# BlueAnon/BD-BNN

Measured on AMD Instinct MI355X. Metric: train_images_per_sec, higher is better.
Workload: dtype bf16; 1 GPU; model=resnet18_bdbnn, global_batch=2048, image=3x224x224, kurtosis=True, parallelism=dp1

## Files before the change

### bdbnn_amd/csrc/api.h

```cpp
#pragma once
#include <hip/hip_runtime.h>
#include <cstdint>

constexpr int BDBNN_MAX_TENSORS = 64;

struct TensorListArg {
  const float* ptr[BDBNN_MAX_TENSORS];
  int64_t numel[BDBNN_MAX_TENSORS];
  int n;
};

struct PtrList { float* ptr[BDBNN_MAX_TENSORS]; };

constexpr int64_t BDBNN_CHUNK_ELEMS = 32 * 1024;

constexpr int bdbnn_bn_sum_rows(int act_kind) {
  return act_kind == 3 ? 4 : 3;
}

extern "C" {

void bdbnn_sign_pack(const void* x, uint32_t* out, int64_t pixels, int C,
                     int CW, bool bf16, hipStream_t stream);
void bdbnn_binsign_decode(const void* x, void* y, int64_t n, bool in_bf16,
// ... 91 lines not shown
                             int64_t n, int C, int act_kind, bool bf16,
                             hipStream_t stream);
void bdbnn_bn_fold_sums(const float* sums32, float* sums, int n,
                        hipStream_t stream);
void bdbnn_bn_act_bwd_apply(const void* dy, const void* z, const void* x,
                            const float* mean, const float* invstd,
                            const float* gamma, const float* a,
                            const float* sums, void* dx, void* dskip,
                            int64_t n, int C, int act_kind, float inv_n,
                            bool bf16, hipStream_t stream);
void bdbnn_bn_act_eval(const void* x, const void* skip, const float* rm,
                       const float* rv, const float* gamma,
                       const float* beta, const float* a, const float* b1,
                       const float* b2, void* out, int64_t n, int C,
                       int act_kind, float eps, bool bf16,
                       hipStream_t stream);
void bdbnn_bn_fold(const float* gamma, const float* beta, const float* rm,
                   const float* rv, const float* b1, float* sc, float* sh,
                   int C, float eps, hipStream_t stream);

void bdbnn_bn_relu_maxpool_fwd(
    const void* x, const float* mean, const float* invstd,
    const float* gamma, const float* beta, void* out, unsigned char* idx,
    uint32_t* xpk, uint32_t* mpk, int N, int C, int H, int W, int Ho, int Wo,
    int ks, int stride, int pad, bool bf16, hipStream_t stream);
void bdbnn_bn_relu_maxpool_bwd_reduce(
    const void* dy, const unsigned char* idx, const void* x,
    const float* mean, const float* invstd, const float* gamma,
    const float* beta, float* sums32, float* sums, int N, int C, int H,
    int W, int Ho, int Wo, int ks, int stride, int pad, bool bf16,
    hipStream_t stream);
void bdbnn_bn_relu_maxpool_bwd_apply(
    const void* dy, const unsigned char* idx, const void* x,
    const float* mean, const float* invstd, const float* gamma,
    const float* beta, const float* sums, void* dx, int N, int C, int H,
    int W, int Ho, int Wo, int ks, int stride, int pad, bool bf16,
    hipStream_t stream);

int bdbnn_dgrad2_supported(int H, int W, int C, int K);
int bdbnn_conv_dgrad2(const void* g, const void* wd, const uint32_t* mp,
                      const void* x, void* dx, const void* accp, int mode,
                      float t, float k, int N, int H, int W, int C, int K,
                      hipStream_t stream);
void bdbnn_dgrad_wdec(const uint32_t* wp, const float* alpha, void* wd,
                      int C, int K, int nt, hipStream_t stream);
int bdbnn_wgrad2_nslab(int N, int H, int W, int C, int K);
int bdbnn_conv_wgrad2(const void* g, const uint64_t* xcp, float* dwT, int N,
                      int H, int W, int C, int K, hipStream_t stream);
void bdbnn_repack_cplane(const uint32_t* xp, uint64_t* xcp, int NH, int W,
                         int C, int CW, bool parity, hipStream_t stream);
void bdbnn_wgrad_finish(const float* dwT, const float* w, float* dw, int C,
                        int K, int T, int nslab, hipStream_t stream);

int bdbnn_s2_kernels_can_run(int H, int W, int C, int K, int ks);
int bdbnn_dgrad2_s2_supported(int H, int W, int C, int K, int ks);
int bdbnn_conv_dgrad2_s2(const void* g, const void* wd, const uint32_t* mp,
                         const void* x, void* dx, const void* accp, int ks,
                         int mode, float t, float k, int N, int H, int W,
                         int C, int K, hipStream_t stream);
int bdbnn_wgrad2_s2_nslab(int N, int H, int W, int C, int K, int ks);
int bdbnn_conv_wgrad2_s2(const void* g, const uint64_t* planes, float* dwT,
                         int ks, int N, int H, int W, int C, int K,
                         hipStream_t stream);

void bdbnn_kurtosis_fwd(const TensorListArg* lists,
                        const int* block_tensor_dev,
                        const int64_t* block_off_dev, int n_blocks,
                        double* mom_dev, const float* targets, float* stats,
                        float* losses, float* kurts, hipStream_t stream);
void bdbnn_kurtosis_bwd(const TensorListArg* lists, const PtrList* gp,
                        const int* block_tensor_dev,
                        const int64_t* block_off_dev, int n_blocks,
                        const float* stats, const float* targets,
                        const float* gscale, hipStream_t stream);

void bdbnn_weight_kd_fwd(const TensorListArg* meta, const PtrList* ws,
                         const PtrList* wt, const int* bt, const int64_t* bo,
                         int n_blocks, double* out, hipStream_t stream);
void bdbnn_weight_kd_bwd(const TensorListArg* meta, const PtrList* wt,
                         const PtrList* grads, const int* bt,
                         const int64_t* bo, int n_blocks,
                         const float* gscale, hipStream_t stream);

void bdbnn_fused_sgd(const TensorListArg* meta, const PtrList* p,
                     const PtrList* g, const PtrList* buf, const int* bt,
                     const int64_t* bo, int n_blocks, float lr,
                     float momentum, float wd, hipStream_t stream);
void bdbnn_fused_adam(const TensorListArg* meta, const PtrList* p,
                      const PtrList* g, const PtrList* m1, const PtrList* m2,
                      const int* bt, const int64_t* bo, int n_blocks,
                      float lr, float beta1, float beta2, float eps,
                      float wd, float bc1, float bc2, hipStream_t stream);

}
```

### bdbnn_amd/csrc/bind.cpp

```cpp
#include <torch/extension.h>
#include <c10/hip/HIPStream.h>
#include <hip/hip_runtime.h>

#include <atomic>
#include <string>
#include <unordered_map>
#include <utility>
#include <vector>

#include "api.h"

namespace {

hipStream_t cur_stream() {
  return c10::hip::getCurrentHIPStream().stream();
}

bool is_bf16(const at::Tensor& t) { return t.scalar_type() == at::kBFloat16; }

void check_vec8(const at::Tensor& t, bool vec8_c, const char* name,
                const char* who) {
  TORCH_CHECK(t.is_cuda() && (t.scalar_type() == at::kBFloat16 ||
                              t.scalar_type() == at::kFloat),
              who, ": ", name, " must be a bf16 or fp32 CUDA tensor");
// ... 1138 lines not shown
                who, ": mask bitplane [...P...][C/32]");
  } else {
    check_act_bf16_cl(*x, N, C, H, W, who);
  }
  TORCH_CHECK(bdbnn_dgrad2_supported(H, W, (int)C, K) != 0, who,
              ": unsupported shape");
  at::Tensor ac = acc_as_bf16_cl(acc, N, C, H, W, who);
  auto dx = empty_dx(g, N, C, H, W);
  int rc = bdbnn_conv_dgrad2(
      g.data_ptr(), wd.data_ptr(),
      mp ? (const uint32_t*)mp->data_ptr<int>() : nullptr,
      x ? x->data_ptr() : nullptr, dx.data_ptr(),
      ac.defined() ? ac.data_ptr() : nullptr, (int)mode, (float)t, (float)k,
      N, H, W, (int)C, K, cur_stream());
  TORCH_CHECK(rc == 0, who, ": launch rejected the shape");
  return dx;
}

at::Tensor conv_dgrad2(const at::Tensor& g, const at::Tensor& wd,
                       const at::Tensor& mp, int64_t C,
                       const c10::optional<at::Tensor>& acc) {
  return conv_dgrad2_impl(g, wd, &mp, nullptr, C, 0, 0.0, 0.0, acc,
                          "conv_dgrad2");
}

at::Tensor conv_dgrad2_x(const at::Tensor& g, const at::Tensor& wd,
                         const at::Tensor& x, int64_t C, int64_t mode,
                         double t, double k,
                         const c10::optional<at::Tensor>& acc) {
  TORCH_CHECK(mode == 1 || mode == 2,
              "conv_dgrad2_x: mode must be 1 (approx) or 2 (EDE)");
  return conv_dgrad2_impl(g, wd, nullptr, &x, C, mode, t, k, acc,
                          "conv_dgrad2_x");
}

at::Tensor conv_wgrad2(const at::Tensor& g, const at::Tensor& xcp,
                       int64_t C) {
  check_grad_bf16_cl(g, "conv_wgrad2");
  int N = (int)g.size(0), K = (int)g.size(1);
  int H = (int)g.size(2), W = (int)g.size(3);
  TORCH_CHECK(xcp.dim() == 2 && xcp.size(0) == C &&
                  xcp.size(1) == (int64_t)N * H,
              "conv_wgrad2: c-plane bitplanes [C][N*H]");
  TORCH_CHECK(C % 64 == 0 && K % 64 == 0 && W <= 64,
              "conv_wgrad2: unsupported shape");
  int nslab = bdbnn_wgrad2_nslab(N, H, W, (int)C, K);
  TORCH_CHECK(nslab > 0, "conv_wgrad2: unsupported shape");
  auto dwT = at::empty({nslab, 9, C, K}, g.options().dtype(at::kFloat));
  int rc = bdbnn_conv_wgrad2(g.data_ptr(),
                             (const uint64_t*)xcp.data_ptr<int64_t>(),
                             dwT.data_ptr<float>(), N, H, W, (int)C, K,
                             cur_stream());
  TORCH_CHECK(rc == 0, "conv_wgrad2: launch rejected the shape");
  return dwT;
}


static bool s2_dims_sane(int64_t H, int64_t W, int64_t C, int64_t K) {
  return H >= 1 && W >= 1 && H <= (1 << 20) && C <= (1 << 20) &&
         K <= (1 << 20);
}
static bool dgrad2_s2_ok(int64_t H, int64_t W, int64_t C, int64_t K,
                         int64_t ks) {
  return s2_dims_sane(H, W, C, K) &&
         bdbnn_s2_kernels_can_run((int)H, (int)W, (int)C, (int)K,
                                  (int)ks) != 0;
}
static bool dgrad2_s2_routed(int64_t H, int64_t W, int64_t C, int64_t K,
                             int64_t ks) {
  return s2_dims_sane(H, W, C, K) &&
         bdbnn_dgrad2_s2_supported((int)H, (int)W, (int)C, (int)K,
                                   (int)ks) != 0;
}

at::Tensor conv_dgrad2_s2(const at::Tensor& g, const at::Tensor& wd,
                          int64_t H, int64_t W, int64_t C, int64_t mode,
                          const c10::optional<at::Tensor>& mp,
                          const c10::optional<at::Tensor>& x, double t,
                          double k, const c10::optional<at::Tensor>& acc) {
  const char* who = "conv_dgrad2_s2";
  check_grad_bf16_cl(g, who);
  int N = (int)g.size(0), K = (int)g.size(1);
  TORCH_CHECK(wd.is_cuda() && wd.dim() == 3 &&
                  wd.scalar_type() == at::kBFloat16 && wd.is_contiguous(),
              "conv_dgrad2_s2: wd must be contiguous bf16 [ks*ks][C][K]");
  TORCH_CHECK(wd.size(0) == 9 || wd.size(0) == 1,
              "conv_dgrad2_s2: wd.size(0) must be 9 (3x3) or 1 (1x1)");
  int ks = wd.size(0) == 9 ? 3 : 1;
  TORCH_CHECK(wd.size(1) == C && wd.size(2) == K,
              "conv_dgrad2_s2: wd must be [ks*ks][C][K] for this g and C");
  TORCH_CHECK(dgrad2_s2_ok(H, W, C, K, ks),
              "conv_dgrad2_s2: unsupported shape (H, W, C, K, ks)");
  int64_t Ho = (H + 1) / 2, Wo = (W + 1) / 2;
  TORCH_CHECK(g.size(2) == Ho && g.size(3) == Wo,
              "conv_dgrad2_s2: g spatial size must be the (Ho, Wo) implied "
              "by (H, W, ks)");
  TORCH_CHECK(mode >= 0 && mode <= 2,
              "conv_dgrad2_s2: mode must be 0 (clip-STE), 1 (approx) or 2 "
              "(EDE)");
  const uint32_t* mp_ptr = nullptr;
  const void* x_ptr = nullptr;
  if (mode == 0) {
    TORCH_CHECK(mp.has_value() && !x.has_value(),
                "conv_dgrad2_s2: mode 0 needs mp and x=None");
    TORCH_CHECK(mp->is_cuda() && mp->scalar_type() == at::kInt &&
                    mp->is_contiguous() && mp->size(-1) == C / 32 &&
// ... 198 lines not shown
  m.def("maxpool_bwd", &maxpool_bwd, "gather-based NHWC maxpool bwd");
  m.def("prelu_fwd", &prelu_fwd, "fused NHWC per-channel PReLU fwd");
  m.def("prelu_bwd", &prelu_bwd, "fused NHWC per-channel PReLU bwd");
  m.def("bn_act_fwd_train", &bn_act_fwd_train,
        "fused BN(+add)(+act) training forward -> [out, z, mean, invstd(, "
        "xpk, mpk)]; act_kind 3 (RPReLU) takes b1, b2 and stores u = z + b1 "
        "as z",
        py::arg("x"), py::arg("skip"), py::arg("gamma"), py::arg("beta"),
        py::arg("a"), py::arg("running_mean"), py::arg("running_var"),
        py::arg("momentum"), py::arg("eps"), py::arg("act_kind"),
        py::arg("pre_s1"), py::arg("pre_s2"), py::arg("want_pack"),
        py::arg("b1") = py::none(), py::arg("b2") = py::none());
  m.def("bn_act_bwd", &bn_act_bwd,
        "fused BN(+add)(+act) backward -> [dx, dskip, dgamma, dbeta, da]; "
        "act_kind 3 appends db1, db2");
  m.def("bn_act_eval", &bn_act_eval, "fused BN(+add)(+act) eval forward",
        py::arg("x"), py::arg("skip"), py::arg("gamma"), py::arg("beta"),
        py::arg("a"), py::arg("rm"), py::arg("rv"), py::arg("eps"),
        py::arg("act_kind"), py::arg("b1") = py::none(),
        py::arg("b2") = py::none());
  m.def("bn_relu_maxpool_fwd_train", &bn_relu_maxpool_fwd_train,
        "fused BN + ReLU + maxpool training forward -> [out, idx, mean, "
        "invstd(, xpk, mpk)]",
        py::arg("x"), py::arg("gamma"), py::arg("beta"),
        py::arg("running_mean"), py::arg("running_var"),
        py::arg("momentum"), py::arg("eps"), py::arg("ks"),
        py::arg("stride"), py::arg("pad"), py::arg("pre_s1") = py::none(),
        py::arg("pre_s2") = py::none(), py::arg("want_pack") = false);
  m.def("bn_relu_maxpool_bwd", &bn_relu_maxpool_bwd,
        "fused BN + ReLU + maxpool backward -> [dx, dgamma, dbeta]");
  m.def("conv_dgrad2", &conv_dgrad2,
        "MFMA bf16 dgrad v2: halo-staged 9-tap implicit GEMM with fused "
        "clip-STE mask (3x3/s1/p1); optional acc adds a same-shape "
        "skip-gradient tensor in the epilogue",
        py::arg("g"), py::arg("wd"), py::arg("mp"), py::arg("C"),
        py::arg("acc") = py::none());
  m.def("conv_dgrad2_x", &conv_dgrad2_x,
        "conv_dgrad2 with a value mask of the saved bf16 activation x in "
        "the epilogue: mode 1 = ReAct polynomial, 2 = EDE(t, k)",
        py::arg("g"), py::arg("wd"), py::arg("x"), py::arg("C"),
        py::arg("mode"), py::arg("t"), py::arg("k"),
        py::arg("acc") = py::none());
  m.def("dgrad_weight_decode", &dgrad_weight_decode,
        "packed bits -> mirrored transposed +-alpha bf16 [9][C][K]");
  m.def("dgrad2_supported",
        [](int64_t H, int64_t W, int64_t C, int64_t K) {
          return bdbnn_dgrad2_supported((int)H, (int)W, (int)C, (int)K) !=
                 0;
        },
        "shape support predicate for conv_dgrad2");
  m.def("conv_wgrad2", &conv_wgrad2,
        "MFMA bf16 wgrad v2: all-9-tap block GEMM from sign BITS "
        "(3x3/s1/p1) -> fp32 [9][C][K]");
  m.def("repack_cplane", &repack_cplane,
        "activation sign bits -> padded per-channel u64 row planes");
  m.def("wgrad_finish", &wgrad_finish,
        "dwT transpose to [K][C][3][3] + |w|<=1 STE mask, one pass");
  m.def("dgrad2_s2_supported",
        [](int64_t H, int64_t W, int64_t C, int64_t K, int64_t ks) {
          return dgrad2_s2_routed(H, W, C, K, ks);
        },
        "routing predicate of the stride-2 MFMA backward; H, W are the "
        "input (dx) size, ks in {3 (pad 1), 1 (pad 0)}; false also for "
        "the shapes the kernels run but lose on (3x3 with C >= 128 and "
        "K >= 256)",
        py::arg("H"), py::arg("W"), py::arg("C"), py::arg("K"),
        py::arg("ks"));
  m.def("conv_dgrad2_s2", &conv_dgrad2_s2,
        "MFMA bf16 dgrad of a 3x3/s2/p1 (wd [9][C][K]) or 1x1/s2/p0 (wd "
        "[1][C][K]) binary conv by pixel parity; mode 0 masks with the "
        "bitplane mp, modes 1/2 with the value mask of x; optional acc "
        "adds a same-shape skip-gradient tensor in the epilogue",
        py::arg("g"), py::arg("wd"), py::arg("H"), py::arg("W"),
        py::arg("C"), py::arg("mode"), py::arg("mp"), py::arg("x"),
        py::arg("t"), py::arg("k"), py::arg("acc") = py::none());
  m.def("dgrad_weight_decode_1x1", &dgrad_weight_decode_1x1,
        "packed 1x1 bits -> transposed +-alpha bf16 [1][C][K]");
  m.def("repack_cplane_s2", &repack_cplane_s2,
        "activation sign bits -> per-channel u64 row planes split by "
        "column parity (even columns low word, odd columns high word)",
        py::arg("xp"), py::arg("C"), py::arg("H"), py::arg("W"));
  m.def("conv_wgrad2_s2", &conv_wgrad2_s2,
        "MFMA bf16 wgrad of a 3x3/s2/p1 or 1x1/s2/p0 binary conv from the "
        "parity planes -> fp32 [nslab][ks*ks][C][K]",
        py::arg("g"), py::arg("planes"), py::arg("C"), py::arg("H"),
        py::arg("W"), py::arg("ks"));
  m.def("wgrad_finish_s2", &wgrad_finish_s2,
        "dwT slab sum + transpose to [K][C][ks][ks] + |w|<=1 STE mask");
  m.def("kurtosis_fwd", &kurtosis_fwd, "fused multi-tensor kurtosis fwd");
  m.def("kurtosis_bwd", &kurtosis_bwd, "fused multi-tensor kurtosis bwd");
  m.def("weight_kd_fwd", &weight_kd_fwd, "fused weight-space KD fwd");
  m.def("weight_kd_bwd", &weight_kd_bwd, "fused weight-space KD bwd");
  m.def("fused_sgd", &fused_sgd, "fused multi-tensor SGD-momentum step");
  m.def("fused_adam", &fused_adam, "fused multi-tensor Adam step");
}
```

### bdbnn_amd/csrc/conv_bwd.hip

```cpp
#include "conv_bwd_common.h"

#define DG2_BM 256
#define DG2_BN 64
#define DG2_BK 64

struct Dgrad2Params {
  int N, H, W, C, K;
  int bands_per_image;
  int total_slots;
  int CW;
};

template <int WP, int RB, int GB, bool ACC, int MODE>
__global__ __launch_bounds__(512, 2) void conv_dgrad2_kernel(
    const __bf16* __restrict__ g, const __bf16* __restrict__ wd,
    const uint32_t* __restrict__ mp, __bf16* __restrict__ dx,
    const __bf16* __restrict__ accp, const __bf16* __restrict__ xin,
    float et, float ek,
    Dgrad2Params p, int grid_m, int nb_m, int tiles_per_block) {
  constexpr int WH = WP + 2;
  constexpr int NHE = GB * (RB + 2) * WH;
  constexpr int PIECES = NHE * 8;
  constexpr int PPT = (PIECES + 511) / 512;

// ... 284 lines not shown
                                 float t, float k, int N, int H, int W,
                                 int C, int K, hipStream_t stream) {
  if (mode == 0)
    return dgrad2_launch<0>(g, wd, mp, dx, accp, nullptr, 0.f, 0.f, N, H, W,
                            C, K, stream);
  if (mode == 1)
    return dgrad2_launch<1>(g, wd, nullptr, dx, accp, x, 0.f, 0.f, N, H, W,
                            C, K, stream);
  if (mode == 2)
    return dgrad2_launch<2>(g, wd, nullptr, dx, accp, x, t, k, N, H, W, C,
                            K, stream);
  return -2;
}

template <int NT>
__global__ void dgrad_wdec_kernel(const uint32_t* __restrict__ wp,
                                  const float* __restrict__ alpha,
                                  __bf16* __restrict__ wd, int C, int K,
                                  int CW) {
  int64_t total = (int64_t)NT * C * (K / 8);
  GRID_STRIDE(i, total) {
    int k8 = int(i % (K / 8));
    int64_t rem = i / (K / 8);
    int c = NT == 1 ? int(rem) : int(rem % C);
    int t = NT == 1 ? 0 : int(rem / C);
    int tm = NT - 1 - t;
    int cw = c >> 5, cb = c & 31;
    __bf16 v[8];
#pragma unroll
    for (int j = 0; j < 8; ++j) {
      int k = k8 * 8 + j;
      uint32_t bits = wp[((int64_t)k * NT + tm) * CW + cw];
      float al = alpha[k];
      v[j] = (__bf16)((bits >> cb) & 1 ? -al : al);
    }
    *(uint4*)&wd[((int64_t)t * C + c) * K + k8 * 8] = *(uint4*)v;
  }
}

extern "C" void bdbnn_dgrad_wdec(const uint32_t* wp, const float* alpha,
                                 void* wd, int C, int K, int nt,
                                 hipStream_t stream) {
  int64_t total = (int64_t)nt * C * (K / 8);
  int blocks = (int)bd_min<int64_t>((total + 255) / 256, 4096);
  if (nt == 9)
    dgrad_wdec_kernel<9><<<blocks, 256, 0, stream>>>(wp, alpha, (__bf16*)wd,
                                                     C, K, C / 32);
  else
    dgrad_wdec_kernel<1><<<blocks, 256, 0, stream>>>(wp, alpha, (__bf16*)wd,
                                                     C, K, C / 32);
}


#define WG2_CHUNK 128
#define WG2_BC 64
#define WG2_BK 64

struct Wgrad2Params {
  int N, H, W, C, K;
  int bands_per_image;
  int total_slots;
  int total_chunks;
  int split;
  int nh_rows;
};

template <int WP, int RB, int GB>
__global__ __launch_bounds__(512, 2) void conv_wgrad2_kernel(
    const __bf16* __restrict__ g, const uint64_t* __restrict__ xcp,
    float* __restrict__ dwT, Wgrad2Params p, int grid_ck) {
  constexpr int XROWS = RB + 2;
  constexpr int XSTRIDE = GB * XROWS * WP + 8;
  constexpr int GSTRIDE = WG2_CHUNK + 8;
  constexpr int LGWP = WP == 8 ? 3 : WP == 16 ? 4 : WP == 32 ? 5 : 6;
  constexpr bool RING = (GB == 1);

  const int tid = threadIdx.x;
  int wg = blockIdx.x;
  const int ck = wg % grid_ck;
  const int split_id = wg / grid_ck;
  const int c_blk = ck % (p.C / WG2_BC);
  const int k_blk = ck / (p.C / WG2_BC);
  const int c0 = c_blk * WG2_BC, k0 = k_blk * WG2_BK;

  __shared__ __align__(16) __bf16 X[3 * WG2_BC * XSTRIDE];
  __shared__ __align__(16) __bf16 gT[2][WG2_BK * GSTRIDE];
  __shared__ __align__(16) __bf16 lut[256][8];
  __shared__ float red[4][32][32];
  constexpr int NBITS = WG2_BC * GB * XROWS;
  __shared__ uint64_t xbits[NBITS];
  __shared__ unsigned char xvalid[NBITS];

  wgrad2_fill_sign_lut(lut, tid);

  const int wid = tid >> 6, lane = tid & 63;
  const int qc = (wid >> 1) & 1, qk = wid & 1, ms_grp = wid >> 2;
  const int lrow = lane & 31, lhalf = lane >> 5;

  f32x16 acc[9];
#pragma unroll
  for (int t = 0; t < 9; ++t)
#pragma unroll
    for (int i = 0; i < 16; ++i) acc[t][i] = 0.f;

  const int cpb = (p.total_chunks + p.split - 1) / p.split;
  const int ch_lo = split_id * cpb;
  const int ch_hi = bd_min(ch_lo + cpb, p.total_chunks);
  const int n_chunks = ch_hi - ch_lo;
  int ch = ch_lo;

  const int sg_m = tid >> 2;
  const int sg_k16 = (tid & 3) * 16;
  uint4 greg[2];

#define G_LOAD(chunk)                                                     \
  {                                                                       \
    int band = sg_m / (RB * WP);                                          \
    int rem = sg_m - band * (RB * WP);                                    \
// ... 142 lines not shown
    const int y0m = RING ? u_pb[0] : 0;
    __syncthreads();
    if (cont) X_DECODE(ch, 2, RB)
    else X_DECODE(ch, 0, XROWS)
    if (more) {
      CHUNK_INFO(ch + 1);
      if (cont_n) BITS_LOAD(ch + 1, 2, RB)
      else BITS_LOAD(ch + 1, 0, XROWS)
      G_LOAD(ch + 1);
    }
    __syncthreads();

#pragma unroll
    for (int msl = 0; msl < 4; ++msl) {
      const int m16 = ms_grp * 64 + msl * 16;
      bf16x8 bfrag =
          *(const bf16x8*)&gT[gb][b_k * GSTRIDE + m16 + lhalf * 8];
      const int mstart = m16 + lhalf * 8;
      const int rl = mstart >> LGWP;
      const int band = rl / RB, rloc = rl - band * RB;
      const int xs = mstart & (WP - 1);
      int pl[3];
#pragma unroll
      for (int dy = 0; dy < 3; ++dy) {
        int v = RING ? y0m + rloc + dy : rloc + dy;
        if (RING && v >= XROWS) v -= XROWS;
        if (RING && v >= XROWS) v -= XROWS;
        pl[dy] = band * XROWS + v;
      }
#pragma unroll
      for (int t = 0; t < 9; ++t) {
        const int dy = t / 3, dxs = t - dy * 3;
        bf16x8 afrag = *(const bf16x8*)&X[(dxs * WG2_BC + a_c) * XSTRIDE +
                                          pl[dy] * WP + xs];
        acc[t] =
            __builtin_amdgcn_mfma_f32_32x32x16_bf16(afrag, bfrag, acc[t],
                                                    0, 0, 0);
      }
    }
    __syncthreads();
    if (more) {
      if (cont_n) BITS_WRITE(ch + 1, 2, RB)
      else BITS_WRITE(ch + 1, 0, XROWS)
      G_WRITE(gb ^ 1);
    }
    gb ^= 1;
    ++ch;
  }

  wgrad2_combine_store<9>(acc, red, dwT + (int64_t)split_id * 9 * p.C * p.K,
                          p.C, p.K, c0, k0, wid, lane);
}

template <class F>
static int wgrad2_class(int H, int W, F f) {
  if (W <= 8 && H <= 8) return f(BwdClass<8, 8, 2>{});
  if (W <= 16) return f(BwdClass<16, 8, 1>{});
  if (W <= 32) return f(BwdClass<32, 4, 1>{});
  return f(BwdClass<64, 2, 1>{});
}

static bool wgrad2_shape_ok(int W, int C, int K) {
  return !(C % 64 || K % 64 || W > 64);
}

template <class G>
static Wgrad2Params wgrad2_params(G, int N, int H, int W, int C, int K) {
  Wgrad2Params p;
  p.N = N; p.H = H; p.W = W; p.C = C; p.K = K;
  p.nh_rows = N * H;
  p.bands_per_image = (H + G::RB - 1) / G::RB;
  p.total_slots = N * p.bands_per_image;
  p.total_chunks = (p.total_slots + G::GB - 1) / G::GB;
  int grid_ck = (C / WG2_BC) * (K / WG2_BK);
  p.split = bd_min((256 + grid_ck - 1) / grid_ck, p.total_chunks);
  return p;
}

extern "C" int bdbnn_wgrad2_nslab(int N, int H, int W, int C, int K) {
  if (!wgrad2_shape_ok(W, C, K)) return -1;
  return wgrad2_class(H, W, [&](auto cls) {
    return wgrad2_params(cls, N, H, W, C, K).split;
  });
}

extern "C" int bdbnn_conv_wgrad2(const void* g, const uint64_t* xcp,
                                 float* dwT, int N, int H, int W, int C,
                                 int K, hipStream_t stream) {
  if (!wgrad2_shape_ok(W, C, K)) return -1;
  return wgrad2_class(H, W, [&](auto cls) {
    using G = decltype(cls);
    Wgrad2Params p = wgrad2_params(cls, N, H, W, C, K);
    int grid_ck = (C / WG2_BC) * (K / WG2_BK);
    dim3 grid(grid_ck * p.split);
    conv_wgrad2_kernel<G::WP, G::RB, G::GB><<<grid, 512, 0, stream>>>(
        (const __bf16*)g, xcp, dwT, p, grid_ck);
    return 0;
  });
}

template <bool PARITY>
__global__ void repack_cplane_kernel(const uint32_t* __restrict__ xp,
                                     uint64_t* __restrict__ xcp, int NH,
                                     int W, int C, int CW) {
  GRID_STRIDE(i, (int64_t)NH * CW) {
    int cw = int(i % CW);
    int64_t row = i / CW;
    const uint32_t* src = xp + (row * W) * CW + cw;
    uint64_t acc[32];
#pragma unroll
    for (int c = 0; c < 32; ++c) acc[c] = 0;
    for (int x = 0; x < W; ++x) {
      uint32_t word = src[(int64_t)x * CW];
      int pos = PARITY ? (x >> 1) + ((x & 1) << 5) : x;
#pragma unroll
      for (int c = 0; c < 32; ++c)
        acc[c] |= (uint64_t)((word >> c) & 1) << pos;
    }
#pragma unroll
    for (int c = 0; c < 32; ++c) {
      int cc = cw * 32 + c;
      if (cc < C) xcp[(int64_t)cc * NH + row] = acc[c];
    }
  }
}

extern "C" void bdbnn_repack_cplane(const uint32_t* xp, uint64_t* xcp,
                                    int NH, int W, int C, int CW,
                                    bool parity, hipStream_t stream) {
  int64_t total = (int64_t)NH * CW;
  int blocks = (int)bd_min<int64_t>((total + 255) / 256, 8192);
// ... 40 lines not shown
```

### bdbnn_amd/csrc/conv_bwd_common.h

```cpp
#pragma once
#include "common.h"
#include "act_masks.h"

typedef __attribute__((ext_vector_type(8))) __bf16 bf16x8;
typedef __attribute__((ext_vector_type(16))) float f32x16;

template <int WPV, int RBV, int GBV>
struct BwdClass {
  static constexpr int WP = WPV, RB = RBV, GB = GBV;
};

__device__ __forceinline__ int mfma32_cd_row(int reg, int half) {
  return (reg & 3) + 8 * (reg >> 2) + 4 * half;
}

__device__ __forceinline__ void wgrad2_fill_sign_lut(__bf16 (*lut)[8],
                                                     int tid) {
  for (int b = tid; b < 256; b += 512) {
#pragma unroll
    for (int j = 0; j < 8; ++j)
      lut[b][j] = (__bf16)(((b >> j) & 1) ? 1.f : -1.f);
  }
}

template <int NT>
__device__ __forceinline__ void wgrad2_combine_store(
    const f32x16 (&acc)[NT], float (*red)[32][32], float* __restrict__ slab,
    int C, int K, int c0, int k0, int wid, int lane) {
  const int quad = wid & 3, ms_grp = wid >> 2;
  const int qc = (wid >> 1) & 1, qk = wid & 1;
  const int lrow = lane & 31, lhalf = lane >> 5;
#pragma unroll
  for (int t = 0; t < NT; ++t) {
    __syncthreads();
    if (ms_grp == 1) {
#pragma unroll
      for (int reg = 0; reg < 16; ++reg)
        red[quad][mfma32_cd_row(reg, lhalf)][lrow] = acc[t][reg];
    }
    __syncthreads();
    if (ms_grp == 0) {
#pragma unroll
      for (int reg = 0; reg < 16; ++reg) {
        int row = mfma32_cd_row(reg, lhalf);
        float v = acc[t][reg] + red[quad][row][lrow];
        slab[((int64_t)t * C + c0 + qc * 32 + row) * K + k0 + qk * 32 +
             lrow] = v;
      }
    }
  }
}

template <int MODE>
__device__ __forceinline__ float dgrad2_value_mask(float x, float et,
                                                   float ekt) {
  static_assert(MODE == 1 || MODE == 2, "value mask: mode 1 or 2");
  if constexpr (MODE == 1) {
    return react_poly_mask(x);
  }
  float e = __expf(-2.f * fabsf(et * x));
  float d = 1.f + e;
  return ekt * __fdividef(4.f * e, d * d);
}
```

### bdbnn_amd/ops/binary_conv.py

```python

import os

import torch
import torch.nn as nn
import torch.nn.functional as F

from .binarize import binsign, weight_scale
from .. import _C

_CONV_STATS = os.environ.get("BDBNN_CONV_STATS", "0") == "1"
_MFMA_BWD = os.environ.get("BDBNN_MFMA_BWD", "1") != "0"
_MFMA_BWD_S2 = os.environ.get("BDBNN_MFMA_BWD_S2", "1") != "0"


def _act_grad_mask(x: torch.Tensor, mode: str, t, k) -> torch.Tensor:
    if t is not None and k is not None:
        th = torch.tanh(float(t) * x)
        return float(k) * float(t) * (1.0 - th * th)
    if mode == "approx":
        neg = (x >= -1) & (x < 0)
        pos = (x >= 0) & (x < 1)
        g = torch.zeros_like(x)
        g = torch.where(neg, 2.0 + 2.0 * x, g)
        g = torch.where(pos, 2.0 - 2.0 * x, g)
        return g
    return (x.abs() <= 1).to(x.dtype)


def _owned_route(nat, *, g_dtype, x_dtype, stride, padding, ks, H_in, W_in,
                 H_out, W_out, C, K, mask_mode, valmask):
    if not _MFMA_BWD or (valmask and mask_mode == 0):
        return None
    if g_dtype != torch.bfloat16 or x_dtype != torch.bfloat16:
        return None
    if (ks, stride, padding) == (3, 1, 1):
        return "s1" if nat.dgrad2_supported(H_out, W_out, C, K) else None
    if _MFMA_BWD_S2 and stride == 2 and (ks, padding) in ((3, 1), (1, 0)):
        return "s2" if nat.dgrad2_s2_supported(H_in, W_in, C, K, ks) else None
    return None


def _owned_backward(nat, route, g, w, xp, wp, alpha, C, mode, mp, x, t, k,
                    acc):
    s2 = route == "s2"
    H, W, ks = xp.shape[1], xp.shape[2], w.shape[2]
    wd = (nat.dgrad_weight_decode_1x1 if ks == 1
          else nat.dgrad_weight_decode)(wp, alpha, C)
    if s2:
        dx = nat.conv_dgrad2_s2(g, wd, H, W, C, mode, mp, x, t, k, acc)
        planes = nat.repack_cplane_s2(xp, C, H, W)
        dwT = nat.conv_wgrad2_s2(g, planes, C, H, W, ks)
        dw = nat.wgrad_finish_s2(dwT, w.float())
    else:
        dx = (nat.conv_dgrad2(g, wd, mp, C, acc) if mode == 0
              else nat.conv_dgrad2_x(g, wd, x, C, mode, t, k, acc))
        planes = nat.repack_cplane(xp, C, W)
        dwT = nat.conv_wgrad2(g, planes, C)
        dw = nat.wgrad_finish(dwT, w.float())
    return dx, dw


def _conv_backward(g, xb, wb, stride, padding):
    return torch.ops.aten.convolution_backward(
        g, xb, wb, None, [stride, stride], [padding, padding], [1, 1], False,
        [0, 0], 1, [True, True, False])[:2]


def _packed_fallback(nat, g, w, xp, mp, wp, alpha, C, x_dtype, stride,
                     padding):
    bf16 = g.dtype == torch.bfloat16
    xb = nat.decode_packed(xp, C, bf16)
    wb = nat.weight_decode(wp, alpha, C, bf16)
    dxb, dwb = _conv_backward(g, xb, wb, stride, padding)
    dx = nat.mask_mul_packed(dxb, mp, C, x_dtype == torch.bfloat16)
    return dx, nat.ste_mask_mul(dwb, w, 0, 0.0, 0.0)


def _value_fallback(g, x, w, stride, padding, act_mode, t, k):
    if not x.is_cuda:
        dxb, dwb = _conv_backward(g, binsign(x), weight_scale(w) * binsign(w),
                                  stride, padding)
        return (dxb * _act_grad_mask(x, act_mode, t, k),
                dwb * (w.abs() <= 1).to(w.dtype))
    nat = _C.native_required()
    xb = nat.binsign_decode(x, 1 if g.dtype == torch.bfloat16 else 0)
    wb = (weight_scale(w) * binsign(w)).to(g.dtype)
    dxb, dwb = _conv_backward(g, xb, wb, stride, padding)
    if t is not None and k is not None:
        mode_id, t, k = 2, float(t), float(k)
    else:
        mode_id, t, k = {"ste": 0, "approx": 1}[act_mode], 0.0, 0.0
    return (nat.ste_mask_mul(dxb, x, mode_id, t, k),
            nat.ste_mask_mul(dwb, w, 0, 0.0, 0.0))


class BinaryConvFunction(torch.autograd.Function):

    @staticmethod
    def forward(ctx, x, w, stride, padding, act_mode, t, k,
                want_stats=False, xp_pre=None, mp_pre=None, skip_cell=None):
        ctx.stride = stride
        ctx.padding = padding
        ctx.act_mode = act_mode
        ctx.t = t
        ctx.k = k
        ctx.packed = False
        ctx.valmask = False
        ctx.skip_cell = skip_cell
        if x.is_cuda:
            nat = _C.native_required()
# ... 154 lines not shown
```

### setup.py

```python

import os

from setuptools import setup

os.environ.setdefault("PYTORCH_ROCM_ARCH", "gfx950")

from torch.utils.cpp_extension import BuildExtension, CUDAExtension

ROOT = os.path.dirname(os.path.abspath(__file__))
CSRC = os.path.join(ROOT, "bdbnn_amd", "csrc")

sources = [os.path.join(CSRC, f) for f in (
    "bind.cpp",
    "pack.hip",
    "prelu.hip",
    "bn_act.hip",
    "bn_pool.hip",
    "pool.hip",
    "loss.hip",
    "conv_bwd.hip",
    "conv_bwd_s2.hip",
    "stem_conv.hip",
    "xnor_conv.hip",
    "xnor_conv_mfma.hip",
    "kurtosis.hip",
    "kd.hip",
    "optim.hip",
)]

setup(
    name="bdbnn_amd_native",
    ext_modules=[
        CUDAExtension(
            name="bdbnn_amd._native",
            sources=sources,
            extra_compile_args={
                "cxx": ["-O3", "-std=c++17"],
                "nvcc": ["-O3", "-std=c++17"],
            },
        )
    ],
    cmdclass={"build_ext": BuildExtension.with_options(no_python_abi_suffix=False)},
)
```

Before: 27670 images/s.

## Add pipelined wgrad v3 kernel reading NHWC sign plane with transposed LDS reads

Adds a new MFMA weight-gradient kernel for 3x3 stride-1 binary convs. It reads the packed NHWC sign bits directly, which removes the separate repack_cplane pass. It double-buffers the gradient tiles and the activation ring so global loads overlap MFMA work, and it uses ds_read_tr16 transposed LDS reads with a swizzled layout. Shared wgrad2 helpers move to the common header, and the new route is on by default for all supported widths. The cost is more LDS and register pressure in a new, untested kernel.

```diff
diff --git a/bdbnn_amd/csrc/api.h b/bdbnn_amd/csrc/api.h
--- a/bdbnn_amd/csrc/api.h
+++ b/bdbnn_amd/csrc/api.h
@@ -167,6 +167,11 @@
 void bdbnn_wgrad_finish(const float* dwT, const float* w, float* dw, int C,
                         int K, int T, int nslab, hipStream_t stream);
 
+int bdbnn_wgrad3_supported(int H, int W, int C, int K);
+int bdbnn_wgrad3_nslab(int N, int H, int W, int C, int K);
+int bdbnn_conv_wgrad3(const void* g, const uint32_t* xp, float* dwT, int N,
+                      int H, int W, int C, int K, hipStream_t stream);
+
 int bdbnn_s2_kernels_can_run(int H, int W, int C, int K, int ks);
 int bdbnn_dgrad2_s2_supported(int H, int W, int C, int K, int ks);
 int bdbnn_conv_dgrad2_s2(const void* g, const void* wd, const uint32_t* mp,
diff --git a/bdbnn_amd/csrc/bind.cpp b/bdbnn_amd/csrc/bind.cpp
--- a/bdbnn_amd/csrc/bind.cpp
+++ b/bdbnn_amd/csrc/bind.cpp
@@ -1214,6 +1214,29 @@
                              dwT.data_ptr<float>(), N, H, W, (int)C, K,
                              cur_stream());
   TORCH_CHECK(rc == 0, "conv_wgrad2: launch rejected the shape");
+  return dwT;
+}
+
+at::Tensor conv_wgrad3(const at::Tensor& g, const at::Tensor& xp,
+                       int64_t C) {
+  check_grad_bf16_cl(g, "conv_wgrad3");
+  int N = (int)g.size(0), K = (int)g.size(1);
+  int H = (int)g.size(2), W = (int)g.size(3);
+  TORCH_CHECK(C >= 64 && C % 64 == 0 && K % 64 == 0 && W <= 64,
+              "conv_wgrad3: unsupported shape");
+  TORCH_CHECK(xp.is_cuda() && xp.dim() == 4 &&
+                  xp.scalar_type() == at::kInt && xp.is_contiguous() &&
+                  xp.size(0) == N && xp.size(1) == H && xp.size(2) == W &&
+                  xp.size(3) == C / 32,
+              "conv_wgrad3: xp must be contiguous int32 [N][H][W][C/32]");
+  int nslab = bdbnn_wgrad3_nslab(N, H, W, (int)C, K);
+  TORCH_CHECK(nslab > 0, "conv_wgrad3: unsupported shape");
+  auto dwT = at::empty({nslab, 9, C, K}, g.options().dtype(at::kFloat));
+  int rc = bdbnn_conv_wgrad3(g.data_ptr(),
+                             (const uint32_t*)xp.data_ptr<int>(),
+                             dwT.data_ptr<float>(), N, H, W, (int)C, K,
+                             cur_stream());
+  TORCH_CHECK(rc == 0, "conv_wgrad3: launch rejected the shape");
   return dwT;
 }
 
@@ -1518,6 +1541,16 @@
   m.def("conv_wgrad2", &conv_wgrad2,
         "MFMA bf16 wgrad v2: all-9-tap block GEMM from sign BITS "
         "(3x3/s1/p1) -> fp32 [9][C][K]");
+  m.def("conv_wgrad3", &conv_wgrad3,
+        "MFMA bf16 wgrad v3: pipelined all-9-tap block GEMM from the NHWC "
+        "sign plane, transposed LDS reads (3x3/s1/p1) -> fp32 "
+        "[nslab][9][C][K]");
+  m.def("wgrad3_supported",
+        [](int64_t H, int64_t W, int64_t C, int64_t K) {
+          return bdbnn_wgrad3_supported((int)H, (int)W, (int)C, (int)K) !=
+                 0;
+        },
+        "shape predicate of the conv_wgrad3 route");
   m.def("repack_cplane", &repack_cplane,
         "activation sign bits -> padded per-channel u64 row planes");
   m.def("wgrad_finish", &wgrad_finish,
diff --git a/bdbnn_amd/csrc/conv_bwd.hip b/bdbnn_amd/csrc/conv_bwd.hip
--- a/bdbnn_amd/csrc/conv_bwd.hip
+++ b/bdbnn_amd/csrc/conv_bwd.hip
@@ -360,18 +360,6 @@
 }
 
 
-#define WG2_CHUNK 128
-#define WG2_BC 64
-#define WG2_BK 64
-
-struct Wgrad2Params {
-  int N, H, W, C, K;
-  int bands_per_image;
-  int total_slots;
-  int total_chunks;
-  int split;
-  int nh_rows;
-};
 
 template <int WP, int RB, int GB>
 __global__ __launch_bounds__(512, 2) void conv_wgrad2_kernel(
@@ -620,31 +608,6 @@
                           p.C, p.K, c0, k0, wid, lane);
 }
 
-template <class F>
-static int wgrad2_class(int H, int W, F f) {
-  if (W <= 8 && H <= 8) return f(BwdClass<8, 8, 2>{});
-  if (W <= 16) return f(BwdClass<16, 8, 1>{});
-  if (W <= 32) return f(BwdClass<32, 4, 1>{});
-  return f(BwdClass<64, 2, 1>{});
-}
-
-static bool wgrad2_shape_ok(int W, int C, int K) {
-  return !(C % 64 || K % 64 || W > 64);
-}
-
-template <class G>
-static Wgrad2Params wgrad2_params(G, int N, int H, int W, int C, int K) {
-  Wgrad2Params p;
-  p.N = N; p.H = H; p.W = W; p.C = C; p.K = K;
-  p.nh_rows = N * H;
-  p.bands_per_image = (H + G::RB - 1) / G::RB;
-  p.total_slots = N * p.bands_per_image;
-  p.total_chunks = (p.total_slots + G::GB - 1) / G::GB;
-  int grid_ck = (C / WG2_BC) * (K / WG2_BK);
-  p.split = bd_min((256 + grid_ck - 1) / grid_ck, p.total_chunks);
-  return p;
-}
-
 extern "C" int bdbnn_wgrad2_nslab(int N, int H, int W, int C, int K) {
   if (!wgrad2_shape_ok(W, C, K)) return -1;
   return wgrad2_class(H, W, [&](auto cls) {
diff --git a/bdbnn_amd/csrc/conv_bwd_common.h b/bdbnn_amd/csrc/conv_bwd_common.h
--- a/bdbnn_amd/csrc/conv_bwd_common.h
+++ b/bdbnn_amd/csrc/conv_bwd_common.h
@@ -51,6 +51,44 @@
   }
 }
 
+#define WG2_CHUNK 128
+#define WG2_BC 64
+#define WG2_BK 64
+
+struct Wgrad2Params {
+  int N, H, W, C, K;
+  int bands_per_image;
+  int total_slots;
+  int total_chunks;
+  int split;
+  int nh_rows;
+};
+
+template <class F>
+static int wgrad2_class(int H, int W, F f) {
+  if (W <= 8 && H <= 8) return f(BwdClass<8, 8, 2>{});
+  if (W <= 16) return f(BwdClass<16, 8, 1>{});
+  if (W <= 32) return f(BwdClass<32, 4, 1>{});
+  return f(BwdClass<64, 2, 1>{});
+}
+
+static inline bool wgrad2_shape_ok(int W, int C, int K) {
+  return !(C % 64 || K % 64 || W > 64);
+}
+
+template <class G>
+static Wgrad2Params wgrad2_params(G, int N, int H, int W, int C, int K) {
+  Wgrad2Params p;
+  p.N = N; p.H = H; p.W = W; p.C = C; p.K = K;
+  p.nh_rows = N * H;
+  p.bands_per_image = (H + G::RB - 1) / G::RB;
+  p.total_slots = N * p.bands_per_image;
+  p.total_chunks = (p.total_slots + G::GB - 1) / G::GB;
+  int grid_ck = (C / WG2_BC) * (K / WG2_BK);
+  p.split = bd_min((256 + grid_ck - 1) / grid_ck, p.total_chunks);
+  return p;
+}
+
 template <int MODE>
 __device__ __forceinline__ float dgrad2_value_mask(float x, float et,
                                                    float ekt) {
diff --git a/bdbnn_amd/csrc/conv_wgrad3.hip b/bdbnn_amd/csrc/conv_wgrad3.hip
--- /dev/null
+++ b/bdbnn_amd/csrc/conv_wgrad3.hip
@@ -0,0 +1,263 @@
+#include "conv_bwd_common.h"
+
+typedef __attribute__((ext_vector_type(4))) short wg3_s16x4;
+typedef __attribute__((ext_vector_type(8))) short wg3_s16x8;
+
+__device__ __forceinline__ int wg3_off(int pix, int cb) {
+  return pix * 128 + (cb ^ ((pix & 2) << 5));
+}
+
+__device__ __forceinline__ wg3_s16x4 wg3_tr_read(const char* base, int off) {
+  return __builtin_amdgcn_ds_read_tr16_b64_v4i16(
+      (__attribute__((address_space(3))) wg3_s16x4*)(base + off));
+}
+
+__device__ __forceinline__ bf16x8 wg3_frag(wg3_s16x4 lo, wg3_s16x4 hi) {
+  wg3_s16x8 v = __builtin_shufflevector(lo, hi, 0, 1, 2, 3, 4, 5, 6, 7);
+  return __builtin_bit_cast(bf16x8, v);
+}
+
+template <int WP, int RB, int GB>
+__device__ __forceinline__ void wg3_chunk_mfma(
+    f32x16 (&acc)[9], const char* X, const char* Gs, int pb, int ms_grp,
+    int lhalf, int tq, int a_cb, int b_cb) {
+  constexpr int WR = RB + 2, XW = WP + 2;
+  constexpr int XPL = GB == 1 ? 2 * RB + 4 : 2 * GB * WR;
+  constexpr int LGWP = WP == 8 ? 3 : WP == 16 ? 4 : WP == 32 ? 5 : 6;
+#pragma unroll
+  for (int msl = 0; msl < 4; ++msl) {
+    const int mrun = ms_grp * 64 + msl * 16 + lhalf * 8;
+    const int boff = wg3_off(mrun + tq, b_cb);
+    bf16x8 bfrag = wg3_frag(wg3_tr_read(Gs, boff),
+                            wg3_tr_read(Gs, boff + 4 * 128));
+    const int rl = mrun >> LGWP;
+    const int band = rl / RB, rloc = rl - band * RB;
+    const int xq = (mrun & (WP - 1)) + tq;
+#pragma unroll
+    for (int dy = 0; dy < 3; ++dy) {
+      int plane = pb + band * WR + rloc + dy;
+      if (plane >= XPL) plane -= XPL;
+      const int pix0 = plane * XW + xq;
+#pragma unroll
+      for (int dxs = 0; dxs < 3; ++dxs) {
+        const int aoff = wg3_off(pix0 + dxs, a_cb);
+        bf16x8 afrag = wg3_frag(wg3_tr_read(X, aoff),
+                                wg3_tr_read(X, aoff + 4 * 128));
+        acc[dy * 3 + dxs] = __builtin_amdgcn_mfma_f32_32x32x16_bf16(
+            afrag, bfrag, acc[dy * 3 + dxs], 0, 0, 0);
+      }
+    }
+  }
+}
+
+template <int WP, int RB, int GB>
+__global__ __launch_bounds__(512, 2) void conv_wgrad3_kernel(
+    const __bf16* __restrict__ g, const uint32_t* __restrict__ xp32,
+    float* __restrict__ dwT, Wgrad2Params p, int grid_ck) {
+  constexpr int WR = RB + 2;
+  constexpr int XW = WP + 2;
+  constexpr bool RING = (GB == 1);
+  constexpr int XPL = RING ? 2 * RB + 4 : 2 * GB * WR;
+  constexpr int LGWP = WP == 8 ? 3 : WP == 16 ? 4 : WP == 32 ? 5 : 6;
+  constexpr int XITEMS = GB * WR * XW * 2;
+  constexpr int XIT = (XITEMS + 511) / 512;
+
+  const int tid = threadIdx.x;
+  const int wg = bd_xcd_remap(blockIdx.x, gridDim.x);
+  const int ck = wg % grid_ck;
+  const int split_id = wg / grid_ck;
+  const int c_blk = ck % (p.C / WG2_BC);
+  const int k_blk = ck / (p.C / WG2_BC);
+  const int c0 = c_blk * WG2_BC, k0 = k_blk * WG2_BK;
+
+  __shared__ __align__(16) char X[XPL * XW * 128];
+  __shared__ __align__(16) char G[2][WG2_CHUNK * 128];
+  __shared__ __align__(16) __bf16 lut[256][8];
+  __shared__ float red[4][32][32];
+
+  wgrad2_fill_sign_lut(lut, tid);
+
+  const int wid = tid >> 6, lane = tid & 63;
+  const int qc = (wid >> 1) & 1, qk = wid & 1, ms_grp = wid >> 2;
+  const int lhalf = lane >> 5;
+  const int tq = (lane & 15) >> 2, tp = lane & 3, tgrp = (lane >> 4) & 1;
+  const int a_cb = (qc * 32 + tgrp * 16 + tp * 4) * 2;
+  const int b_cb = (qk * 32 + tgrp * 16 + tp * 4) * 2;
+
+  f32x16 acc[9];
+#pragma unroll
+  for (int t = 0; t < 9; ++t)
+#pragma unroll
+    for (int i = 0; i < 16; ++i) acc[t][i] = 0.f;
+
+  const int cpb = (p.total_chunks + p.split - 1) / p.split;
+  const int ch_lo = split_id * cpb;
+  const int ch_hi = bd_min(ch_lo + cpb, p.total_chunks);
+  const int n_chunks = ch_hi - ch_lo;
+  int ch = ch_lo;
+
+  const int sg_m = tid >> 2;
+  const int sg_k16 = (tid & 3) * 16;
+  uint4 gregA[2];
+
+  int u_n[GB], u_y0[GB];
+  bool u_vs[GB];
+#define CHUNK_INFO(chunk)                                                 \
+  {                                                                       \
+    _Pragma("unroll")                                                     \
+    for (int b = 0; b < GB; ++b) {                                        \
+      int slot = (chunk)*GB + b;                                          \
+      u_vs[b] = slot < p.total_slots;                                     \
+      int n = slot / p.bands_per_image;                                   \
+      u_n[b] = n;                                                         \
+      u_y0[b] = (slot - n * p.bands_per_image) * RB;                      \
+    }                                                                     \
+  }
+
+#define G_LOAD(greg)                                                      \
+  {                                                                       \
+    int band = sg_m / (RB * WP);                                          \
+    int rem = sg_m - band * (RB * WP);                                    \
+    int x = rem & (WP - 1);                                               \
+    uint4 z{0, 0, 0, 0};                                                  \
+    greg[0] = z; greg[1] = z;                                             \
+    if (u_vs[band] && x < p.W) {                                          \
+      int y = u_y0[band] + (rem >> LGWP);                                 \
+      if (y < p.H) {                                                      \
+        const __bf16* src =                                               \
+            g + ((int64_t)(u_n[band] * p.H + y) * p.W + x) * p.K + k0 +   \
+            sg_k16;                                                       \
+        greg[0] = *(const uint4*)src;                                     \
+        greg[1] = *(const uint4*)(src + 8);                               \
+      }                                                                   \
+    }                                                                     \
+  }
+#define G_WRITE(buf, greg)                                                \
+  {                                                                       \
+    char* dst = G[buf] + wg3_off(sg_m, sg_k16 * 2);                       \
+    *(uint4*)dst = greg[0];                                               \
+    *(uint4*)(dst + 16) = greg[1];                                        \
+  }
+
+  int xwA[XIT], xoA[XIT];
+  const int cw = p.C / 32;
+#define XB_LOAD(r0, NR, pbase, xw, xo)                                    \
+  {                                                                       \
+    _Pragma("unroll")                                                     \
+    for (int it = 0; it < XIT; ++it) {                                    \
+      int i = tid + it * 512;                                             \
+      int v = 0, o = -1;                                                  \
+      if (i < GB * (NR) * XW * 2) {                                       \
+        int h = i & 1, px = i >> 1;                                       \
+        int col = px % XW;                                                \
+        int rem = px / XW;                                                \
+        int w = (r0) + rem % (NR);                                        \
+        int band = rem / (NR);                                            \
+        int x = col - 1, y = u_y0[band] + w - 1;                          \
+        int plane = (pbase) + band * WR + w;                              \
+        if (plane >= XPL) plane -= XPL;                                   \
+        o = wg3_off(plane * XW + col, h * 64);                            \
+        if (u_vs[band] && x >= 0 && x < p.W && y >= 0 && y < p.H) {       \
+          v = xp32[((int64_t)(u_n[band] * p.H + y) * p.W + x) * cw +      \
+                   (c0 >> 5) + h];                                        \
+          o |= 1;                                                         \
+        }                                                                 \
+      }                                                                   \
+      xw[it] = v;                                                         \
+      xo[it] = o;                                                         \
+    }                                                                     \
+  }
+#define XB_WRITE(xw, xo)                                                  \
+  {                                                                       \
+    _Pragma("unroll")                                                     \
+    for (int it = 0; it < XIT; ++it) {                                    \
+      if (xo[it] >= 0) {                                                  \
+        char* dst = X + (xo[it] & ~1);                                    \
+        const bool on = xo[it] & 1;                                       \
+        _Pragma("unroll")                                                 \
+        for (int jj = 0; jj < 4; ++jj) {                                  \
+          uint4 vv{0, 0, 0, 0};                                           \
+          if (on)                                                         \
+            vv = *(const uint4*)&lut[((unsigned)xw[it] >> (8 * jj)) &     \
+                                     255u][0];                            \
+          *(uint4*)(dst + jj * 16) = vv;                                  \
+        }                                                                 \
+      }                                                                   \
+    }                                                                     \
+  }
+
+#define IS_CONT(chunk) \
+  (RING && (chunk) > ch_lo && ((chunk) % p.bands_per_image) != 0)
+#define PB_NEXT(pbprev, chunk)                                            \
+  (((pbprev) + (IS_CONT(chunk) ? RB : GB * WR)) % XPL)
+#define LOADS(chunk, pbase, greg, xw, xo)                                 \
+  {                                                                       \
+    CHUNK_INFO(chunk);                                                    \
+    if (IS_CONT(chunk)) XB_LOAD(2, RB, pbase, xw, xo)                     \
+    else XB_LOAD(0, WR, pbase, xw, xo)                                    \
+    G_LOAD(greg);                                                         \
+  }
+
+  int pb0 = 0, pb1 = 0;
+  if (n_chunks > 0) {
+    LOADS(ch, 0, gregA, xwA, xoA);
+    __syncthreads();
+    XB_WRITE(xwA, xoA);
+    G_WRITE(0, gregA);
+  }
+  int gb = 0;
+
+  for (int ci = 0; ci < n_chunks; ++ci) {
+    __syncthreads();
+    if (ci + 1 < n_chunks) {
+      pb1 = PB_NEXT(pb0, ch + 1);
+      LOADS(ch + 1, pb1, gregA, xwA, xoA);
+    }
+    wg3_chunk_mfma<WP, RB, GB>(acc, X, G[gb], pb0, ms_grp, lhalf, tq, a_cb,
+                               b_cb);
+    if (ci + 1 < n_chunks) {
+      XB_WRITE(xwA, xoA);
+      G_WRITE(gb ^ 1, gregA);
+    }
+    gb ^= 1;
+    pb0 = pb1;
+    ++ch;
+  }
+
+  wgrad2_combine_store<9>(acc, red, dwT + (int64_t)split_id * 9 * p.C * p.K,
+                          p.C, p.K, c0, k0, wid, lane);
+}
+
+static bool wgrad3_class_routed(int WP) {
+  return WP == 64 || WP == 32 || WP == 16 || WP == 8;
+}
+
+extern "C" int bdbnn_wgrad3_supported(int H, int W, int C, int K) {
+  if (H < 1 || W < 1 || C < 64 || K < 64 || !wgrad2_shape_ok(W, C, K))
+    return 0;
+  return wgrad2_class(H, W, [&](auto cls) {
+    return (int)wgrad3_class_routed(decltype(cls)::WP);
+  });
+}
+
+extern "C" int bdbnn_wgrad3_nslab(int N, int H, int W, int C, int K) {
+  if (!wgrad2_shape_ok(W, C, K)) return -1;
+  return wgrad2_class(H, W, [&](auto cls) {
+    return wgrad2_params(cls, N, H, W, C, K).split;
+  });
+}
+
+extern "C" int bdbnn_conv_wgrad3(const void* g, const uint32_t* xp,
+                                 float* dwT, int N, int H, int W, int C,
+                                 int K, hipStream_t stream) {
+  if (!wgrad2_shape_ok(W, C, K)) return -1;
+  return wgrad2_class(H, W, [&](auto cls) {
+    using G = decltype(cls);
+    Wgrad2Params p = wgrad2_params(cls, N, H, W, C, K);
+    int grid_ck = (C / WG2_BC) * (K / WG2_BK);
+    dim3 grid(grid_ck * p.split);
+    conv_wgrad3_kernel<G::WP, G::RB, G::GB><<<grid, 512, 0, stream>>>(
+        (const __bf16*)g, xp, dwT, p, grid_ck);
+    return 0;
+  });
+}
diff --git a/bdbnn_amd/ops/binary_conv.py b/bdbnn_amd/ops/binary_conv.py
--- a/bdbnn_amd/ops/binary_conv.py
+++ b/bdbnn_amd/ops/binary_conv.py
@@ -11,6 +11,7 @@
 _CONV_STATS = os.environ.get("BDBNN_CONV_STATS", "0") == "1"
 _MFMA_BWD = os.environ.get("BDBNN_MFMA_BWD", "1") != "0"
 _MFMA_BWD_S2 = os.environ.get("BDBNN_MFMA_BWD_S2", "1") != "0"
+_WGRAD3 = os.environ.get("BDBNN_WGRAD3", "1") != "0"
 
 
 def _act_grad_mask(x: torch.Tensor, mode: str, t, k) -> torch.Tensor:
@@ -54,8 +55,11 @@
     else:
         dx = (nat.conv_dgrad2(g, wd, mp, C, acc) if mode == 0
               else nat.conv_dgrad2_x(g, wd, x, C, mode, t, k, acc))
-        planes = nat.repack_cplane(xp, C, W)
-        dwT = nat.conv_wgrad2(g, planes, C)
+        if _WGRAD3 and nat.wgrad3_supported(H, W, C, w.shape[0]):
+            dwT = nat.conv_wgrad3(g, xp, C)
+        else:
+            planes = nat.repack_cplane(xp, C, W)
+            dwT = nat.conv_wgrad2(g, planes, C)
         dw = nat.wgrad_finish(dwT, w.float())
     return dx, dw
 
diff --git a/setup.py b/setup.py
--- a/setup.py
+++ b/setup.py
@@ -20,6 +20,7 @@
     "loss.hip",
     "conv_bwd.hip",
     "conv_bwd_s2.hip",
+    "conv_wgrad3.hip",
     "stem_conv.hip",
     "xnor_conv.hip",
     "xnor_conv_mfma.hip",
```

After: 31480 images/s, median of 6. 13.8% higher.
